# IXarea/LittleGAN

Measured on AMD Instinct MI355X. Metric: 128x128 CelebA-shaped images/sec (G+D+Adj step), higher is better.
Workload: dtype bf16; 1 GPU; C3: 128x128x3 synthetic CelebA, batch 256/GPU, bf16 MFMA conv/transposed-conv + Adjuster branch; global_batch=256, per_gpu_batch=256, image=128, cond_dim=40, parallelism=dp1, launch=eager launches

## Files before the change

include/littlegan_hip.h:

```cpp
#ifndef LITTLEGAN_HIP_H
#define LITTLEGAN_HIP_H
#include <stddef.h>

#ifdef __cplusplus
extern "C" {
#endif

#define LG_ABI_VERSION 1
#define LG_OK 0
#define LG_ERR_ARG (-1)
#define LG_ERR_LAUNCH (-2)
#define LG_ERR_UNSUPPORTED (-3)
#define LG_DT_F32 0
#define LG_DT_BF16 1

int lg_abi_version(void);
const char* lg_last_error(void);
const char* lg_last_kernel(void);
int lg_clear_kernel(void);

size_t lg_conv_pack_bytes(int cb, int cs, int dtype);
int lg_conv_pack(const float* w, void* pack, int cb, int cs, int dtype, void* stream);

int lg_conv2d_s2_fwd(const float* x, const void* pack, const float* bias, float* y, int B, int Hs, int Ws, int cb,
// ... 110 lines not shown
int lg_instnorm_leaky_bwd_drop(const float* x, const float* stats, const void* g, int g_is_bf16, float* dx, void* dx16,
                               float* dgamma, float* dbeta, float* db, int C, void* workspace, size_t ws_bytes, int B,
                               long long L, float alpha, int accumulate, const long long* key, int call, int level, int r0,
                               float rate, void* stream);
int lg_instnorm_leaky_bwd_z16_drop(const void* z16, const float* stats, const void* g, int g_is_bf16, float* dx, void* dx16,
                                   float* dgamma, float* dbeta, float* db, int C, const void* partials, int nparts_in,
                                   void* workspace, size_t ws_bytes, int B, long long L, float alpha, int accumulate,
                                   const long long* key, int call, int level, int r0, float rate, void* stream);

int lg_convT_s1_tanh_bwd_nf(const float* x, const void* x16, const float* dpre, const void* pack, void* dx16, float* dw,
                            float* db, void* workspace, size_t ws_bytes, int B, int H, int W, int cb, int cs, int accumulate,
                            int dtype, const void* z16, const float* stats, float alpha, void* part, size_t part_bytes,
                            int* nparts, void* stream);

int lg_dense_fwd(const float* x, const float* w, const float* bias, float* y, int B, int K, int N, void* stream);
int lg_dense_wgrad(const float* x, const float* dy, float* dw, float* db, int B, int K, int N, int accumulate,
                   void* stream);
int lg_dense_dgrad(const float* dy, const float* w, float* dx, int B, int K, int N, void* stream);
int lg_concat_cols(const float* a, int ka, const float* c, int kc, float* out, int B, void* stream);
int lg_adj_conditions(const float* first, const float* second, float* t, float* u, int B, int c, void* stream);
size_t lg_heads_fwd_workspace_bytes(int B, int K, int c);
int lg_heads_fwd(const float* x, const float* wpr, const float* bpr, const float* wc, const float* bc, float* p,
                 void* workspace, size_t ws_bytes, int B, int K, int c, void* stream);
int lg_heads_dgrad(const float* dz, const float* wpr, const float* wc, float* dx, int B, int K, int c, void* stream);
int lg_heads_wgrad(const float* x, const float* dz, float* dwpr, float* dbpr, float* dwc, float* dbc, int B, int K,
                   int c, int accumulate, void* stream);

int lg_bce_heads_loss_fwd_bwd(const float* p, const float* t_c, float t_pr, float w_pr, float w_c, float* loss,
                              float* dz, int B, int c, int accumulate, void* stream);
size_t lg_l1_workspace_bytes(void);
int lg_l1_tanh_loss_fwd_bwd(const float* t, const float* img, const float* g_in, float* dpre, float* loss,
                            void* workspace, size_t ws_bytes, long long n, float lambda, int accumulate, void* stream);

int lg_clip_adam_update(float* w, const float* g, float* m, float* v, long long n, const float* state, float lr,
                        float b1, float b2, float eps, float clip, float gscale, void* stream);
int lg_adam_advance(float* state, float b1, float b2, void* stream);
int lg_axpby(float* y, const float* x, float a, float b, long long n, void* stream);

int lg_clip_adam_ema_update(float* w, const float* g, float* m, float* v, float* ema, long long n, long long lo, long long hi,
// ... 68 lines not shown
```

littlegan_amd/_lib.py:

```python
from __future__ import annotations

import ctypes as C
import os

_HERE = os.path.dirname(os.path.abspath(__file__))
LIB_PATH = os.path.join(_HERE, "liblittlegan_hip.so")

DT_F32, DT_BF16 = 0, 1

P, I, L, F, Z = C.c_void_p, C.c_int, C.c_longlong, C.c_float, C.c_size_t

SIGNATURES = {
    "lg_abi_version": (I, []),
    "lg_last_error": (C.c_char_p, []),
    "lg_conv_pack_bytes": (Z, [I, I, I]),
    "lg_conv_pack": (I, [P, P, I, I, I, P]),
    "lg_conv2d_s2_fwd": (I, [P, P, P, P, I, I, I, I, I, I, P]),
    "lg_conv_stats_workspace_bytes": (Z, [I, I, I, I, I]),
    "lg_conv_fwd_stats_fused": (I, [I, I, I, I, I, I, I]),
    "lg_conv2d_s2_fwd_stats": (I, [P, P, P, P, P, P, I, I, I, I, I, I, P, Z, P, P]),
    "lg_conv2d_s2_dgrad_m16": (I, [P, P, P, P, P, I, I, I, I, I, I, P]),
    "lg_conv2d_s2_wgrad_m16": (I, [P, P, P, P, P, P, Z, I, I, I, I, I, I, I, P]),
    "lg_conv2d_s2_dgrad": (I, [P, P, P, I, I, I, I, I, I, P]),
    "lg_conv2d_s2_wgrad": (I, [P, P, P, P, Z, I, I, I, I, I, I, I, P]),
# ... 35 lines not shown
    "lg_instnorm_leaky_bwd_z16_p": (I, [P, P, P, I, P, P, P, P, P, I, P, I, P, Z, I, L, I, I, F, I, P]),
    "lg_conv2d_s2_dgrad_nf": (I, [P, P, P, I, I, I, I, I, P, P, F, P, Z, P, P]),
    "lg_convT_s2_dgrad_nf": (I, [P, P, P, I, I, I, I, I, P, P, F, P, Z, P, P]),
    "lg_convT_s2_dgrad_bn_supported": (I, [I, I, I, I, I]),
    "lg_convT_s2_dgrad_bn": (I, [P, P, P, F, P, P, I, I, I, I, I, P, P, F, P, Z, P, P]),
    "lg_instnorm_bwd_coef": (I, [P, P, I, P, I, L, P]),
    "lg_dropout_key": (I, [P, L, L, P]),
    "lg_dropout_mask": (I, [P, I, I, I, I, L, F, P, P]),
    "lg_instnorm_leaky_apply_drop": (I, [P, P, P, P, I, L, F, P, I, I, I, F, P]),
    "lg_instnorm_leaky_apply_z16_drop": (I, [P, P, P, P, I, L, F, P, I, I, I, F, P]),
    "lg_instnorm_leaky_apply_z16_p_drop": (I, [P, P, I, P, P, P, P, P, I, L, F, P, I, I, I, F, P]),
    "lg_instnorm_leaky_bwd_drop": (I, [P, P, P, I, P, P, P, P, P, I, P, Z, I, L, F, I, P, I, I, I, F, P]),
    "lg_instnorm_leaky_bwd_z16_drop": (I, [P, P, P, I, P, P, P, P, P, I, P, I, P, Z, I, L, F, I, P, I, I, I, F, P]),
    "lg_convT_s1_tanh_bwd_nf": (I, [P, P, P, P, P, P, P, P, Z, I, I, I, I, I, I, I, P, P, F, P, Z, P, P]),
    "lg_dense_fwd": (I, [P, P, P, P, I, I, I, P]),
    "lg_dense_wgrad": (I, [P, P, P, P, I, I, I, I, P]),
    "lg_dense_dgrad": (I, [P, P, P, I, I, I, P]),
    "lg_concat_cols": (I, [P, I, P, I, P, I, P]),
    "lg_adj_conditions": (I, [P, P, P, P, I, I, P]),
    "lg_heads_fwd_workspace_bytes": (Z, [I, I, I]),
    "lg_heads_fwd": (I, [P, P, P, P, P, P, P, Z, I, I, I, P]),
    "lg_heads_dgrad": (I, [P, P, P, P, I, I, I, P]),
    "lg_heads_wgrad": (I, [P, P, P, P, P, P, I, I, I, I, P]),
    "lg_bce_heads_loss_fwd_bwd": (I, [P, P, F, F, F, P, P, I, I, I, P]),
    "lg_l1_workspace_bytes": (Z, []),
    "lg_l1_tanh_loss_fwd_bwd": (I, [P, P, P, P, P, P, Z, L, F, I, P]),
    "lg_clip_adam_update": (I, [P, P, P, P, L, P, F, F, F, F, F, F, P]),
    "lg_adam_advance": (I, [P, F, F, P]),
    "lg_axpby": (I, [P, P, F, F, L, P]),
    "lg_clip_adam_ema_update": (I, [P, P, P, P, P, L, L, L, P, P, F, F, F, F, F, F, F, P]),
    "lg_ema_advance": (I, [P, P]),
    "lg_swap_f32": (I, [P, P, L, P]),
    "lg_philox4x32": (I, [P, I, L, L, P]),
    "lg_randn": (I, [P, L, F, F, L, L, P]),
    "lg_augment_workspace_bytes": (Z, [I]),
    "lg_augment": (I, [P, P, I, I, I, P, F, F, F, F, L, L, P, Z, P]),
    "lg_fid_stats_workspace_bytes": (Z, [L, I]),
# ... 70 lines not shown
```

littlegan_amd/csrc/dense.hip:

```cpp
#include "lg_common.h"

namespace {

template <int TB>
__global__ __launch_bounds__(256) void dense_fwd_kernel(const float* __restrict__ x, const float* __restrict__ w,
                                                        const float* __restrict__ bias, float* __restrict__ y, int B,
                                                        int K, int N) {
  extern __shared__ float xs[];
  const int b0 = blockIdx.y * TB;
  for (int i = threadIdx.x; i < TB * K; i += 256) {
    const int b = i / K, k = i - b * K;
    xs[i] = (b0 + b < B) ? x[(long long)(b0 + b) * K + k] : 0.f;
  }
  __syncthreads();
  const int n = (blockIdx.x * 256 + threadIdx.x) * 4;
  if (n >= N) return;
  f32x4 acc[TB];
  const f32x4 bv = bias ? *reinterpret_cast<const f32x4*>(bias + n) : f32x4{0.f, 0.f, 0.f, 0.f};
#pragma unroll
  for (int b = 0; b < TB; ++b) acc[b] = bv;
  for (int k = 0; k < K; ++k) {
    const f32x4 wv = *reinterpret_cast<const f32x4*>(w + (long long)k * N + n);
#pragma unroll
    for (int b = 0; b < TB; ++b) acc[b] += xs[b * K + k] * wv;
// ... 128 lines not shown
  LG_CHECK_ARG(x && w && y, "lg_dense_fwd: null pointer");
  LG_CHECK_ARG(B > 0 && K > 0 && K <= 1024 && N > 0 && N % 4 == 0, "lg_dense_fwd: bad shape B=%d K=%d N=%d", B, K, N);
  {
    const int rc = lg_dense_fwd_mfma_try(x, w, bias, y, B, K, N, stream);
    if (rc != LG_ERR_UNSUPPORTED) return rc;
  }
  constexpr int TB = 8;
  dim3 grid(lg_cdiv(N, 1024), lg_cdiv(B, TB));
  hipLaunchKernelGGL(dense_fwd_kernel<TB>, grid, dim3(256), TB * K * sizeof(float), (hipStream_t)stream, x, w, bias, y,
                     B, K, N);
  LG_CHECK_LAUNCH("lg_dense_fwd");
  lg_note_kernel("dense_fwd_kernel");
  return LG_OK;
}

extern "C" int lg_dense_wgrad(const float* x, const float* dy, float* dw, float* db, int B, int K, int N,
                              int accumulate, void* stream) {
  LG_CHECK_ARG(x && dy && dw, "lg_dense_wgrad: null pointer");
  LG_CHECK_ARG(B > 0 && K > 0 && N > 0 && N % 4 == 0, "lg_dense_wgrad: bad shape B=%d K=%d N=%d", B, K, N);
  {
    const int rc = lg_dense_wgrad_mfma_try(x, dy, dw, db, B, K, N, accumulate, stream);
    if (rc != LG_ERR_UNSUPPORTED) return rc;
  }
  constexpr int KT = 16;
  const size_t lds = ((size_t)((B * KT + 3) / 4) * 4 + (size_t)(KT + 1) * 64 * 4) * sizeof(float);
  LG_CHECK_ARG(lds <= 160 * 1024, "lg_dense_wgrad: batch %d too large for the LDS staging of x", B);
  static bool attr_set = false;
  if (!attr_set) {
    (void)hipFuncSetAttribute(reinterpret_cast<const void*>(dense_wgrad_kernel<KT>), hipFuncAttributeMaxDynamicSharedMemorySize, 160 * 1024);
    attr_set = true;
// ... 17 lines not shown
```

littlegan_amd/csrc/heads.hip:

```cpp
#include "lg_common.h"

namespace {

constexpr int HC_MAX = 40;

__device__ __forceinline__ float head_w(const float* __restrict__ wpr, const float* __restrict__ wc, int k, int j, int c) {
  return j == 0 ? wpr[k] : wc[(long long)k * c + (j - 1)];
}

constexpr int FS = 16;
constexpr int FKC = 256;

__global__ __launch_bounds__(256) void heads_fwd_kernel(const float* __restrict__ x, const float* __restrict__ wpr,
                                                        const float* __restrict__ wc, float* __restrict__ part, int B,
                                                        int K, int c) {
  __shared__ __attribute__((aligned(16))) float xs[FS][FKC];
  __shared__ float sred[4][FS][64];
  const int lane = threadIdx.x & 63, wid = threadIdx.x >> 6;
  const int b0 = blockIdx.y * FS, k0 = blockIdx.x * FKC;
  const bool act = lane <= c;
#pragma unroll
  for (int i = 0; i < FS * FKC / 4 / 256; ++i) {
    const int q = threadIdx.x + 256 * i, b = q / (FKC / 4), k4 = (q % (FKC / 4)) * 4;
    f32x4 v = {0.f, 0.f, 0.f, 0.f};
// ... 25 lines not shown
  for (int i = threadIdx.x; i < FS * 64; i += 256) {
    const int s = i >> 6, j = i & 63;
    if (j <= c && b0 + s < B)
      part[((long long)blockIdx.x * B + b0 + s) * (c + 1) + j] = (sred[0][s][j] + sred[1][s][j]) + (sred[2][s][j] + sred[3][s][j]);
  }
}

__global__ __launch_bounds__(256) void heads_final_kernel(const float* __restrict__ part, const float* __restrict__ bpr,
                                                          const float* __restrict__ bc, float* __restrict__ p, int B,
                                                          int c, int nkc) {
  const int i = blockIdx.x * 256 + threadIdx.x;
  const int n = B * (c + 1);
  if (i >= n) return;
  const int j = i % (c + 1);
  float z = 0.f;
  for (int q = 0; q < nkc; ++q) z += part[(long long)q * n + i];
  z += j == 0 ? bpr[0] : bc[j - 1];
  p[i] = 1.f / (1.f + expf(-z));
}

constexpr int DB = 16;
__global__ __launch_bounds__(256) void heads_dgrad_kernel(const float* __restrict__ dz, const float* __restrict__ wpr,
                                                          const float* __restrict__ wc, float* __restrict__ dx, int B,
                                                          int K, int c) {
  extern __shared__ __attribute__((aligned(16))) float dsm[];
  const int cp = c | 1;
  float* sw = dsm;
  float* sdz = dsm + ((256 * cp + 3) / 4) * 4;
  const int b0 = blockIdx.y * DB, k0 = blockIdx.x * 256;
  const int kn = min(256, K - k0);
  {
// ... 129 lines not shown
                              void* stream) {
  LG_CHECK_ARG(dz && wpr && wc && dx, "lg_heads_dgrad: null pointer");
  LG_CHECK_ARG(B > 0 && K > 0 && c >= 1 && c <= HC_MAX, "lg_heads_dgrad: bad shape B=%d K=%d c=%d", B, K, c);
  {
    const int rc = lg_heads_dgrad_mfma_try(dz, wpr, wc, dx, B, K, c, stream);
    if (rc != LG_ERR_UNSUPPORTED) return rc;
  }
  dim3 grid(lg_cdiv(K, 256), lg_cdiv(B, DB));
  const size_t lds = (size_t)((256 * (c | 1) + 3) / 4 * 4 + DB * (c + 1)) * sizeof(float);
  hipLaunchKernelGGL(heads_dgrad_kernel, grid, dim3(256), lds, (hipStream_t)stream, dz, wpr, wc, dx, B, K, c);
  LG_CHECK_LAUNCH("lg_heads_dgrad");
  lg_note_kernel("heads_dgrad_kernel");
  return LG_OK;
}

extern "C" int lg_heads_wgrad(const float* x, const float* dz, float* dwpr, float* dbpr, float* dwc, float* dbc, int B,
                              int K, int c, int accumulate, void* stream) {
  LG_CHECK_ARG(x && dz && dwpr && dbpr && dwc && dbc, "lg_heads_wgrad: null pointer");
  LG_CHECK_ARG(B > 0 && K > 0 && K % 4 == 0 && c >= 1 && c <= HC_MAX, "lg_heads_wgrad: bad shape B=%d K=%d c=%d", B, K, c);
  {
    const int rc = lg_heads_wgrad_mfma_try(x, dz, dwpr, dbpr, dwc, dbc, B, K, c, accumulate, stream);
    if (rc != LG_ERR_UNSUPPORTED) return rc;
  }
  hipLaunchKernelGGL(heads_wgrad_kernel, dim3(lg_cdiv(K, WK)), dim3(256), 0, (hipStream_t)stream, x, dz, dwpr, dbpr,
                     dwc, dbc, B, K, c, accumulate);
  LG_CHECK_LAUNCH("lg_heads_wgrad");
  lg_note_kernel("heads_wgrad_kernel");
  return LG_OK;
}
```

littlegan_amd/csrc/skinny_mfma.hip:

```cpp
#include <stdlib.h>
#include "lg_common.h"

namespace {

__device__ __forceinline__ f32x16 mfma2(float a, float b, f32x16 c) { return __builtin_amdgcn_mfma_f32_32x32x2f32(a, b, c, 0, 0, 0); }
__device__ __forceinline__ f32x16 zero16() {
  f32x16 z;
#pragma unroll
  for (int e = 0; e < 16; ++e) z[e] = 0.f;
  return z;
}
struct HeadCol { const float* ptr; int stride; bool ok; };
__device__ __forceinline__ HeadCol head_col(const float* wpr, const float* wc, int j, int c) {
  HeadCol h;
  h.ok = j <= c;
  h.ptr = j == 0 ? wpr : wc + (h.ok ? j - 1 : 0);
  h.stride = j == 0 ? 1 : c;
  return h;
}

__global__ __launch_bounds__(256) void heads_fwd_mfma_kernel(const float* __restrict__ x, const float* __restrict__ wpr,
                                                             const float* __restrict__ wc, float* __restrict__ part, int B,
                                                             int K, int c) {
  __shared__ float sred[4][2][16][64];
  const int lane = threadIdx.x & 63, wid = threadIdx.x >> 6, r = lane & 31, h = lane >> 5;
  const int b0 = blockIdx.y * 32, kw = blockIdx.x * 512 + wid * 128 + 8 * h;
  const float* xr = x + (long long)(b0 + r) * K + kw;
  const HeadCol c0 = head_col(wpr, wc, r, c), c1 = head_col(wpr, wc, 32 + r, c);
  const bool two = c >= 32;
  f32x16 acc0 = zero16(), acc1 = zero16();
  constexpr int GU = 2;
  for (int g2 = 0; g2 < 8; g2 += GU) {
    f32x4 alo[GU], ahi[GU];
    float w0[GU][8], w1[GU][8];
// ... 112 lines not shown
    bw[s] = j <= c ? (j == 0 ? wpr[kt + r] : wc[(long long)(kt + r) * c + j - 1]) : 0.f;
  }
  __syncthreads();
  for (int t = 0; t < nmt; ++t) {
    const int mt = blockIdx.y + t * gridDim.y;
    const float* zr = sdz + (t * 32 + r) * cp + h;
    f32x16 acc = zero16();
#pragma unroll
    for (int s = 0; s < SMAX; ++s) acc = mfma2(2 * s + h <= c ? zr[2 * s] : 0.f, bw[s], acc);
    float* o = dx + (long long)(mt * 32 + 4 * h) * K + kt + r;
#pragma unroll
    for (int e = 0; e < 16; ++e) o[(long long)((e & 3) + 8 * (e >> 2)) * K] = acc[e];
  }
}

constexpr int SD = 72;
__global__ __launch_bounds__(256) void dense_fwd_mfma_kernel(const float* __restrict__ x, const float* __restrict__ w,
                                                             const float* __restrict__ bias, float* __restrict__ y, int B,
                                                             int K, int N) {
  extern __shared__ float sx[];
  const int lane = threadIdx.x & 63, wid = threadIdx.x >> 6, r = lane & 31, h = lane >> 5;
  const int n = blockIdx.x * 128 + wid * 32 + r, b0 = blockIdx.y * 32;
  const int nsteps = (K + 1) / 2, kp = K | 1;
  {
    const float* src = x + (long long)b0 * K;
    int row = threadIdx.x / K, col = threadIdx.x - row * K;
    const int dq = 256 / K, dr = 256 - dq * K;
    for (int i = threadIdx.x; i < 32 * K; i += 256) {
      sx[row * kp + col] = src[i];
      row += dq; col += dr;
// ... 10 lines not shown
#pragma unroll 4
  for (int s = 0; s < nsteps; s += 2) {
    const bool ok = 2 * s + h < K, ok2 = 2 * s + 2 + h < K;
    const float a = ok ? xr[2 * s] : 0.f, a2 = ok2 ? xr[2 * s + 2] : 0.f;
    const float b = ok ? wp[(long long)(2 * s) * N] : 0.f, b2 = ok2 ? wp[(long long)(2 * s + 2) * N] : 0.f;
    acc = mfma2(a, b, acc);
    acc2 = mfma2(a2, b2, acc2);
  }
#pragma unroll
  for (int e = 0; e < 16; ++e) acc[e] += acc2[e];
  float* o = y + (long long)(b0 + 4 * h) * N + n;
#pragma unroll
  for (int e = 0; e < 16; ++e) o[(long long)((e & 3) + 8 * (e >> 2)) * N] = acc[e];
}

template <int MT>
__global__ __launch_bounds__(256) void dense_wgrad_mfma_kernel(const float* __restrict__ x, const float* __restrict__ dy,
                                                               float* __restrict__ dw, float* __restrict__ db, int B, int K,
                                                               int N, int accumulate) {
  __shared__ float red[MT][16][64];
  __shared__ float rb[64];
  const int lane = threadIdx.x & 63, wid = threadIdx.x >> 6, r = lane & 31, h = lane >> 5;
  const int n = blockIdx.x * 32 + r;
  const int bq = B / 4, bs = wid * bq;
  f32x16 acc[MT];
#pragma unroll
  for (int m = 0; m < MT; ++m) acc[m] = zero16();
  float bsum = 0.f;
  const float* dp = dy + (long long)(bs + h) * N + n;
  const float* xp = x + (long long)(bs + h) * K + r;
// ... 31 lines not shown
      float* o = dw + (long long)k * N + blockIdx.x * 32 + rr;
      *o = (accumulate ? *o : 0.f) + red[m][e][hh * 32 + rr];
    }
  }
  if (db && threadIdx.x < 32) {
    float* o = db + blockIdx.x * 32 + threadIdx.x;
    *o = (accumulate ? *o : 0.f) + (rb[threadIdx.x] + rb[32 + threadIdx.x]);
  }
}

bool skinny_on() {
  static int on = -1;
  if (on < 0) on = lg_env_flag("LG_NO_SKINNY_MFMA") ? 0 : 1;
  return on == 1;
}

}

extern "C" int lg_heads_fwd_mfma_try(const float* x, const float* wpr, const float* wc, float* part, int B, int K, int c,
                                     int* nkc_out, void* stream) {
  if (!skinny_on() || B % 32 || K % 512 || c < 1 || c > 40) return LG_ERR_UNSUPPORTED;
  hipLaunchKernelGGL(heads_fwd_mfma_kernel, dim3(K / 512, B / 32), dim3(256), 0, (hipStream_t)stream, x, wpr, wc, part, B, K, c);
  LG_CHECK_LAUNCH("lg_heads_fwd(mfma)");
  lg_note_kernel("heads_fwd_mfma_kernel");
  *nkc_out = K / 512;
  return LG_OK;
}

extern "C" int lg_heads_wgrad_mfma_try(const float* x, const float* dz, float* dwpr, float* dbpr, float* dwc, float* dbc, int B,
                                       int K, int c, int accumulate, void* stream) {
  if (!skinny_on() || B % 64 || K % 32 || c < 1 || c > 40) return LG_ERR_UNSUPPORTED;
  hipLaunchKernelGGL(heads_wgrad_mfma_kernel, dim3(K / 32), dim3(256), 0, (hipStream_t)stream, x, dz, dwpr, dbpr, dwc, dbc, B, K, c,
                     accumulate);
  LG_CHECK_LAUNCH("lg_heads_wgrad(mfma)");
  lg_note_kernel("heads_wgrad_mfma_kernel");
  return LG_OK;
}

extern "C" int lg_heads_dgrad_mfma_try(const float* dz, const float* wpr, const float* wc, float* dx, int B, int K, int c,
                                       void* stream) {
  if (!skinny_on() || B % 32 || K % 128 || c < 1 || c > 40) return LG_ERR_UNSUPPORTED;
  const int mt = B / 32, gy = mt >= 8 ? 4 : (mt >= 2 ? 2 : 1);
  const size_t lds = (size_t)((mt + gy - 1) / gy) * 32 * ((c + 1) | 1) * sizeof(float);
  if (lds > 48 * 1024) return LG_ERR_UNSUPPORTED;
  hipLaunchKernelGGL(heads_dgrad_mfma_kernel, dim3(K / 128, gy), dim3(256), lds, (hipStream_t)stream, dz, wpr, wc, dx, B, K, c);
  LG_CHECK_LAUNCH("lg_heads_dgrad(mfma)");
  lg_note_kernel("heads_dgrad_mfma_kernel");
  return LG_OK;
}

extern "C" int lg_dense_fwd_mfma_try(const float* x, const float* w, const float* bias, float* y, int B, int K, int N,
                                     void* stream) {
  if (!skinny_on() || B % 32 || N % 128 || K < 1 || K > 2 * SD) return LG_ERR_UNSUPPORTED;
  hipLaunchKernelGGL(dense_fwd_mfma_kernel, dim3(N / 128, B / 32), dim3(256), (size_t)32 * (K | 1) * sizeof(float),
                     (hipStream_t)stream, x, w, bias, y, B, K, N);
  LG_CHECK_LAUNCH("lg_dense_fwd(mfma)");
  lg_note_kernel("dense_fwd_mfma_kernel");
  return LG_OK;
}

extern "C" int lg_dense_wgrad_mfma_try(const float* x, const float* dy, float* dw, float* db, int B, int K, int N, int accumulate,
                                       void* stream) {
// ... 13 lines not shown
```

littlegan_amd/model.py:

```python
from __future__ import annotations

import math
import zlib
from typing import Dict, List, Optional

import torch

from . import ops
from ._lib import DT_BF16, DT_F32


def _dtype_of(args) -> int:
    name = getattr(args, "mfma_dtype", "f32")
    if name not in ("f32", "bf16"):
        raise ValueError(f"mfma_dtype must be 'f32' or 'bf16', got {name!r}")
    return DT_BF16 if name == "bf16" else DT_F32


def _device_of(args):
    return torch.device(getattr(args, "device", "cuda"))


def _glorot(shape, gen, device):
    if len(shape) == 2:
# ... 114 lines not shown
                st = ops.stats_tensor(st)
                m = h if i == 4 else h16
            else:
                h16 = None
                h = m = ops.instnorm_apply(z, st, None, 0, 1, a, drop=drops[i - 1] if drops else None)
            outs.append(m if tails is None else (m, tails[i - 1]))
            saved.append((x, z, st, x16))
            x, x16, raw = h, h16, None
        if ctx is not None:
            ctx["enc"] = saved
            ctx["enc_maps"] = outs
            ctx["enc_drop"] = drops
        return outs

    def backward(self, ctx, g_last, need_wgrad: bool, need_input_grad: bool, rows: Optional[slice] = None,
                 wgrad_levels=None):
        a = self.args.leaky_alpha
        packs = self.packs()
        drops = ctx.get("enc_drop")
        r0 = 0
        if drops is not None and rows is not None:
            r0, _, step = rows.indices(ctx["enc"][0][1].shape[0])
            if step != 1:
                raise ValueError("Encoder.backward: contiguous row ranges only")
        masked = drops is not None and drops[0].active
        g_h = g_last
        levels = set(range(1, 5)) if (need_wgrad and wgrad_levels is None) else (set(wgrad_levels or ()) if need_wgrad else set())
        lowest = 1 if need_input_grad else (min(levels) if levels else 5)
        any_wgrad = need_wgrad
        nfp = None
        for i in range(4, lowest - 1, -1):
            need_wgrad = any_wgrad and i in levels
            cb, cs = self.chans[i - 1]
            x, z, st, x16 = ctx["enc"][i - 1]
            if need_wgrad and x is None and x16 is None:
                raise ValueError("Encoder.backward: this context was recorded with top_only=True (no normalised inputs kept): "
                                 "it cannot give weight gradients")
            if rows is not None:
                z, st = z[rows], st[rows]
                x = x[rows] if x is not None else None
                x16 = x16[rows] if x16 is not None else None
            dgm = self._g[f"norm{i}.gamma"] if need_wgrad else None
            dbt = self._g[f"norm{i}.beta"] if need_wgrad else None
            want_dx = i > lowest or (i == 1 and need_input_grad)
            m16 = self.dtype == DT_BF16
# ... 212 lines not shown


class _DenseNorm(_Module):

    def __init__(self, args, in_dim):
        super().__init__(args)
        self.in_dim = in_dim
        self.out_dim = args.init_dim ** 2 * args.conv_filter[0]
        self._add("dense.kernel", (in_dim, self.out_dim), "kernel")
        self._add("dense.bias", (self.out_dim,), "zeros")
        self._add("norm.gamma", (1,), "ones")
        self._add("norm.beta", (1,), "zeros")

    def __call__(self, x, ctx: Optional[dict] = None, skip=None, want16: bool = False):
        a = self.args.leaky_alpha
        u = ops.dense_fwd(x, self._w["dense.kernel"], self._w["dense.bias"])
        st = ops.instnorm_stats(u, self._w["norm.gamma"], self._w["norm.beta"], 1, a)
        w16 = torch.empty(u.shape, dtype=torch.bfloat16, device=u.device) if want16 else None
        if isinstance(skip, tuple):
            b1 = skip[0].shape[0]
            w = torch.empty_like(u)
            for lo, hi, sk in ((0, b1, skip[0]), (b1, u.shape[0], skip[1])):
                ops.instnorm_apply(u[lo:hi], st[lo:hi], sk.reshape(hi - lo, -1), 1, 0, a, out=w[lo:hi],
                                   out16=w16[lo:hi] if want16 else None)
        else:
            w = ops.instnorm_apply(u, st, skip.reshape(u.shape) if skip is not None else None, 1, 0, a, out16=w16)
        if ctx is not None:
            ctx["dn"] = (x, u, st)
        shp = (-1, self.args.init_dim, self.args.init_dim, self.args.conv_filter[0])
        return w.view(shp), (w16.view(shp) if want16 else None)

    def backward(self, ctx, g):
# ... 107 lines not shown

    def __call__(self, inputs, ctx: Optional[dict] = None):
        p = self.forward_packed(inputs, ctx)
        return p[:, :1], p[:, 1:]

    def backward(self, ctx, dz, need_wgrad: bool, need_input_grad: bool, rows: Optional[slice] = None, train_range=None):
        lo, hi = train_range if train_range is not None else (0, 20)
        heads = need_wgrad and lo <= 16 and hi >= 20
        levels = [i for i in range(1, 5) if lo <= 4 * (i - 1) and 4 * i <= hi] if need_wgrad else []
        x = ctx["heads_x"] if rows is None else ctx["heads_x"][rows]
        if heads:
            ops.heads_wgrad(x, dz, self._g["dense_pr.kernel"], self._g["dense_pr.bias"], self._g["dense_cond.kernel"],
                            self._g["dense_cond.bias"])
        if not levels and not need_input_grad:
            return None
        dx = ops.heads_dgrad(dz, self._w["dense_pr.kernel"], self._w["dense_cond.kernel"])
        i, f = self.args.init_dim, self.args.conv_filter[0]
        return self.encoder.backward(ctx, dx.view(-1, i, i, f), bool(levels), need_input_grad, rows, wgrad_levels=levels)

    def gradient_penalty(self, image, gp_weight: float, loss=None, gp_loss=None, train_range=None):
        lo, hi = train_range if train_range is not None else (0, 20)
        heads = lo <= 16 and hi >= 20
        levels = [i for i in range(1, 5) if lo <= 4 * (i - 1) and 4 * i <= hi]
        ctx: dict = {}
        p = self.forward_packed(image, ctx)
        B = image.shape[0]
        i, f = self.args.init_dim, self.args.conv_filter[0]
        wpr = self._w["dense_pr.kernel"]
        g_top = ops.gp_heads_seed(p, wpr)
        g0, rec = self.encoder.backward_recorded(ctx, g_top.view(B, i, i, f))
        u0, r = ops.gp_seed(g0, gp_weight, loss, gp_loss)
        u4, uz2 = self.encoder.gp_sweep(ctx, rec, u0, levels, min(levels) if levels else 5)
        _, g2 = ops.gp_heads_2nd(p, wpr, ctx["heads_x"], u4.view(B, -1), dwpr=self._g["dense_pr.kernel"] if heads else None,
# ... 104 lines not shown
```

littlegan_amd/ops.py:

```python
from __future__ import annotations

import torch

from . import _lib
from ._lib import DT_BF16, DT_F32, check

_WS = {}
_WS_RETIRED = []
_WS_PINNED = False
NSTAT = 8


class Profile:
    enabled = False
    records = []
    after_conv = None

    @classmethod
    def start(cls):
        cls.records = []
        cls.enabled = True

    @classmethod
    def stop(cls):
# ... 621 lines not shown
    return out


def dense_fwd(x, w, bias, out=None):
    B, K = x.shape
    N = w.shape[1]
    _chk(x, name="x")
    _chk(w, (K, N), "w")
    if out is None:
        out = torch.empty(B, N, dtype=torch.float32, device=x.device)
    _chk(out, (B, N), "out")
    check(_lib.load().lg_dense_fwd(_p(x), _p(w), _p(bias), _p(out), B, K, N, _stream()), "lg_dense_fwd")
    return out


def dense_wgrad(x, dy, dw, db, accumulate=False):
    B, K = x.shape
    N = dy.shape[1]
    _chk(x, name="x")
    _chk(dy, (B, N), "dy")
    _chk(dw, (K, N), "dw")
    check(_lib.load().lg_dense_wgrad(_p(x), _p(dy), _p(dw), _p(db), B, K, N, int(accumulate), _stream()),
          "lg_dense_wgrad")


def concat_cols(a, c, out=None):
    B, ka = a.shape
    kc = c.shape[1]
    _chk(a, name="a")
    _chk(c, (B, kc), "c")
# ... 39 lines not shown
    ws = workspace(int(lib.lg_heads_fwd_workspace_bytes(B, K, c)), x.device, "small")
    check(lib.lg_heads_fwd(_p(x), _p(wpr), _p(bpr), _p(wc), _p(bc), _p(out), _p(ws), ws.numel(), B, K, c, _stream()),
          "lg_heads_fwd")
    return out


def heads_dgrad(dz, wpr, wc, out=None):
    B = dz.shape[0]
    K, c = wc.shape
    _chk(dz, (B, 1 + c), "dz")
    if out is None:
        out = torch.empty(B, K, dtype=torch.float32, device=dz.device)
    _chk(out, (B, K), "out")
    check(_lib.load().lg_heads_dgrad(_p(dz), _p(wpr), _p(wc), _p(out), B, K, c, _stream()), "lg_heads_dgrad")
    return out


def heads_wgrad(x, dz, dwpr, dbpr, dwc, dbc, accumulate=False):
    B, K = x.shape
    c = dwc.shape[1]
    _chk(x, name="x")
    _chk(dz, (B, 1 + c), "dz")
    _chk(dwpr, (K, 1), "dwpr")
    _chk(dwc, (K, c), "dwc")
    check(_lib.load().lg_heads_wgrad(_p(x), _p(dz), _p(dwpr), _p(dbpr), _p(dwc), _p(dbc), B, K, c, int(accumulate),
                                     _stream()), "lg_heads_wgrad")


def bce_heads_loss(p, t_c, t_pr, w_pr, w_c, loss, dz, accumulate):
    B, J = p.shape
# ... 477 lines not shown
```

Measured before the change: 24290 images/sec.

## Fuse instnorm moments into dense fwd and norm-bwd partials into heads dgrad

Adds a dense forward MFMA kernel that computes per-row leaky/instnorm moment partials (count, mean, M2 in double) in its epilogue, so the generator's first norm no longer needs a separate stats pass. Adds a heads dgrad variant that also reads the bf16 encoder level-4 pre-activation and stats, producing norm-backward partial sums that are passed to the encoder backward. The heads fwd reduction loop is batched into 16-wide loads. The aim is fewer kernel launches and fewer re-reads of activations, at the cost of extra register pressure, double-precision shuffles and new workspaces.

```diff
diff --git a/include/littlegan_hip.h b/include/littlegan_hip.h
--- a/include/littlegan_hip.h
+++ b/include/littlegan_hip.h
@@ -148,6 +148,10 @@
                             int* nparts, void* stream);
 
 int lg_dense_fwd(const float* x, const float* w, const float* bias, float* y, int B, int K, int N, void* stream);
+int lg_dense_fwd_mom_supported(int B, int K, int N);
+size_t lg_dense_fwd_mom_workspace_bytes(int B, int N);
+int lg_dense_fwd_mom(const float* x, const float* w, const float* bias, float* y, int B, int K, int N, float alpha, void* mom,
+                     size_t mom_bytes, int* nparts, void* stream);
 int lg_dense_wgrad(const float* x, const float* dy, float* dw, float* db, int B, int K, int N, int accumulate,
                    void* stream);
 int lg_dense_dgrad(const float* dy, const float* w, float* dx, int B, int K, int N, void* stream);
@@ -157,6 +161,11 @@
 int lg_heads_fwd(const float* x, const float* wpr, const float* bpr, const float* wc, const float* bc, float* p,
                  void* workspace, size_t ws_bytes, int B, int K, int c, void* stream);
 int lg_heads_dgrad(const float* dz, const float* wpr, const float* wc, float* dx, int B, int K, int c, void* stream);
+int lg_set_top_fuse(int on);
+int lg_heads_dgrad_nf_supported(int B, int K, int c, int C);
+size_t lg_heads_dgrad_nf_workspace_bytes(int B, int K);
+int lg_heads_dgrad_nf(const float* dz, const float* wpr, const float* wc, float* dx, int B, int K, int c, int C, const void* z16,
+                      const float* stats, float alpha, void* part, size_t part_bytes, int* nparts, void* stream);
 int lg_heads_wgrad(const float* x, const float* dz, float* dwpr, float* dbpr, float* dwc, float* dbc, int B, int K,
                    int c, int accumulate, void* stream);
 
diff --git a/littlegan_amd/_lib.py b/littlegan_amd/_lib.py
--- a/littlegan_amd/_lib.py
+++ b/littlegan_amd/_lib.py
@@ -73,6 +73,9 @@
     "lg_instnorm_leaky_bwd_z16_drop": (I, [P, P, P, I, P, P, P, P, P, I, P, I, P, Z, I, L, F, I, P, I, I, I, F, P]),
     "lg_convT_s1_tanh_bwd_nf": (I, [P, P, P, P, P, P, P, P, Z, I, I, I, I, I, I, I, P, P, F, P, Z, P, P]),
     "lg_dense_fwd": (I, [P, P, P, P, I, I, I, P]),
+    "lg_dense_fwd_mom_supported": (I, [I, I, I]),
+    "lg_dense_fwd_mom_workspace_bytes": (Z, [I, I]),
+    "lg_dense_fwd_mom": (I, [P, P, P, P, I, I, I, F, P, Z, P, P]),
     "lg_dense_wgrad": (I, [P, P, P, P, I, I, I, I, P]),
     "lg_dense_dgrad": (I, [P, P, P, I, I, I, P]),
     "lg_concat_cols": (I, [P, I, P, I, P, I, P]),
@@ -80,6 +83,10 @@
     "lg_heads_fwd_workspace_bytes": (Z, [I, I, I]),
     "lg_heads_fwd": (I, [P, P, P, P, P, P, P, Z, I, I, I, P]),
     "lg_heads_dgrad": (I, [P, P, P, P, I, I, I, P]),
+    "lg_set_top_fuse": (I, [I]),
+    "lg_heads_dgrad_nf_supported": (I, [I, I, I, I]),
+    "lg_heads_dgrad_nf_workspace_bytes": (Z, [I, I]),
+    "lg_heads_dgrad_nf": (I, [P, P, P, P, I, I, I, I, P, P, F, P, Z, P, P]),
     "lg_heads_wgrad": (I, [P, P, P, P, P, P, I, I, I, I, P]),
     "lg_bce_heads_loss_fwd_bwd": (I, [P, P, F, F, F, P, P, I, I, I, P]),
     "lg_l1_workspace_bytes": (Z, []),
diff --git a/littlegan_amd/csrc/dense.hip b/littlegan_amd/csrc/dense.hip
--- a/littlegan_amd/csrc/dense.hip
+++ b/littlegan_amd/csrc/dense.hip
@@ -166,6 +166,26 @@
   return LG_OK;
 }
 
+extern "C" int lg_dense_fwd_mom_mfma_try(const float* x, const float* w, const float* bias, float* y, int B, int K, int N,
+                                         double* mom, float alpha, void* stream);
+
+extern "C" size_t lg_dense_fwd_mom_workspace_bytes(int B, int N) {
+  if (B <= 0 || N <= 0) return 0;
+  return (size_t)B * (size_t)lg_cdiv(N, 128) * 3 * sizeof(double);
+}
+
+extern "C" int lg_dense_fwd_mom(const float* x, const float* w, const float* bias, float* y, int B, int K, int N, float alpha,
+                                void* mom, size_t mom_bytes, int* nparts, void* stream) {
+  LG_CHECK_ARG(x && w && y && mom && nparts, "lg_dense_fwd_mom: null pointer");
+  LG_CHECK_ARG(B > 0 && K > 0 && K <= 1024 && N > 0 && N % 4 == 0, "lg_dense_fwd_mom: bad shape B=%d K=%d N=%d", B, K, N);
+  LG_CHECK_ARG(mom_bytes >= lg_dense_fwd_mom_workspace_bytes(B, N), "lg_dense_fwd_mom: workspace too small (%zu bytes)", mom_bytes);
+  *nparts = 0;
+  const int rc = lg_dense_fwd_mom_mfma_try(x, w, bias, y, B, K, N, (double*)mom, alpha, stream);
+  if (rc == LG_OK) *nparts = N / 128;
+  if (rc != LG_ERR_UNSUPPORTED) return rc;
+  return lg_dense_fwd(x, w, bias, y, B, K, N, stream);
+}
+
 extern "C" int lg_dense_wgrad(const float* x, const float* dy, float* dw, float* db, int B, int K, int N,
                               int accumulate, void* stream) {
   LG_CHECK_ARG(x && dy && dw, "lg_dense_wgrad: null pointer");
diff --git a/littlegan_amd/csrc/heads.hip b/littlegan_amd/csrc/heads.hip
--- a/littlegan_amd/csrc/heads.hip
+++ b/littlegan_amd/csrc/heads.hip
@@ -63,7 +63,14 @@
   if (i >= n) return;
   const int j = i % (c + 1);
   float z = 0.f;
-  for (int q = 0; q < nkc; ++q) z += part[(long long)q * n + i];
+  for (int q0 = 0; q0 < nkc; q0 += 16) {
+    float v[16];
+#pragma unroll
+    for (int u = 0; u < 16; ++u) v[u] = q0 + u < nkc ? part[(long long)(q0 + u) * n + i] : 0.f;
+#pragma unroll
+    for (int u = 0; u < 16; ++u)
+      if (q0 + u < nkc) z += v[u];
+  }
   z += j == 0 ? bpr[0] : bc[j - 1];
   p[i] = 1.f / (1.f + expf(-z));
 }
@@ -223,6 +230,27 @@
   return LG_OK;
 }
 
+extern "C" int lg_heads_dgrad_nf_mfma_try(const float* dz, const float* wpr, const float* wc, float* dx, int B, int K, int c, int C,
+                                          const void* z16, const float* stats, float alpha, double* part, void* stream);
+
+extern "C" size_t lg_heads_dgrad_nf_workspace_bytes(int B, int K) {
+  if (B <= 0 || K <= 0) return 0;
+  return (size_t)B * (size_t)lg_cdiv(K, 128) * 2 * sizeof(double);
+}
+
+extern "C" int lg_heads_dgrad_nf(const float* dz, const float* wpr, const float* wc, float* dx, int B, int K, int c, int C,
+                                 const void* z16, const float* stats, float alpha, void* part, size_t part_bytes, int* nparts,
+                                 void* stream) {
+  LG_CHECK_ARG(dz && wpr && wc && dx && z16 && stats && part && nparts, "lg_heads_dgrad_nf: null pointer");
+  LG_CHECK_ARG(B > 0 && K > 0 && c >= 1 && c <= HC_MAX && C > 0, "lg_heads_dgrad_nf: bad shape B=%d K=%d c=%d C=%d", B, K, c, C);
+  LG_CHECK_ARG(part_bytes >= lg_heads_dgrad_nf_workspace_bytes(B, K), "lg_heads_dgrad_nf: workspace too small (%zu bytes)", part_bytes);
+  *nparts = 0;
+  const int rc = lg_heads_dgrad_nf_mfma_try(dz, wpr, wc, dx, B, K, c, C, z16, stats, alpha, (double*)part, stream);
+  if (rc == LG_OK) *nparts = K / 128;
+  if (rc != LG_ERR_UNSUPPORTED) return rc;
+  return lg_heads_dgrad(dz, wpr, wc, dx, B, K, c, stream);
+}
+
 extern "C" int lg_heads_wgrad(const float* x, const float* dz, float* dwpr, float* dbpr, float* dwc, float* dbc, int B,
                               int K, int c, int accumulate, void* stream) {
   LG_CHECK_ARG(x && dz && dwpr && dbpr && dwc && dbc, "lg_heads_wgrad: null pointer");
diff --git a/littlegan_amd/csrc/skinny_mfma.hip b/littlegan_amd/csrc/skinny_mfma.hip
--- a/littlegan_amd/csrc/skinny_mfma.hip
+++ b/littlegan_amd/csrc/skinny_mfma.hip
@@ -18,6 +18,22 @@
   h.stride = j == 0 ? 1 : c;
   return h;
 }
+
+
+template <int N>
+__device__ __forceinline__ void rs_step(double (&v)[16], int r, int o) {
+  const bool up = (r & o) != 0;
+#pragma unroll
+  for (int i = 0; i < N; ++i) {
+    const double keep = up ? v[i + N] : v[i], send = up ? v[i] : v[i + N];
+    v[i] = keep + __shfl_xor(send, o, 64);
+  }
+}
+__device__ __forceinline__ double rs16(double (&v)[16], int r) {
+  rs_step<8>(v, r, 16); rs_step<4>(v, r, 8); rs_step<2>(v, r, 4); rs_step<1>(v, r, 2);
+  return v[0] + __shfl_xor(v[0], 1, 64);
+}
+__device__ __forceinline__ int acc_row(int e, int h) { return (e & 3) + 8 * (e >> 2) + 4 * h; }
 
 __global__ __launch_bounds__(256) void heads_fwd_mfma_kernel(const float* __restrict__ x, const float* __restrict__ wpr,
                                                              const float* __restrict__ wc, float* __restrict__ part, int B,
@@ -160,6 +176,78 @@
   }
 }
 
+
+__global__ __launch_bounds__(256) void heads_dgrad_nf_mfma_kernel(const float* __restrict__ dz, const float* __restrict__ wpr,
+                                                                  const float* __restrict__ wc, float* __restrict__ dx, int B,
+                                                                  int K, int c, const unsigned short* __restrict__ z,
+                                                                  const float* __restrict__ stats, double* __restrict__ part,
+                                                                  float alpha) {
+  constexpr int SMAX = 21;
+  extern __shared__ float sdz[];
+  __shared__ f32x4 sst[2][32];
+  __shared__ double sred[2][4][32][2];
+  const int lane = threadIdx.x & 63, wid = threadIdx.x >> 6, r = lane & 31, h = lane >> 5;
+  const int kt = blockIdx.x * 128 + wid * 32;
+  const int cp = (c + 1) | 1, nmt = (B / 32 - blockIdx.y + gridDim.y - 1) / gridDim.y, nparts = K / 128;
+  for (int t = 0; t < nmt; ++t) {
+    const float* src = dz + (long long)(blockIdx.y + t * gridDim.y) * 32 * (c + 1);
+    for (int i = threadIdx.x; i < 32 * (c + 1); i += 256) {
+      const int row = i / (c + 1), j = i - row * (c + 1);
+      sdz[(t * 32 + row) * cp + j] = src[i];
+    }
+  }
+  float bw[SMAX];
+#pragma unroll
+  for (int s = 0; s < SMAX; ++s) {
+    const int j = 2 * s + h;
+    bw[s] = j <= c ? (j == 0 ? wpr[kt + r] : wc[(long long)(kt + r) * c + j - 1]) : 0.f;
+  }
+  if (threadIdx.x < 32) {
+    const float* sp = stats + (long long)(blockIdx.y * 32 + threadIdx.x) * 8;
+    sst[0][threadIdx.x] = f32x4{sp[0], sp[4], sp[2], sp[3]};
+  }
+  __syncthreads();
+  for (int t = 0; t < nmt; ++t) {
+    const int mt = blockIdx.y + t * gridDim.y, pb = t & 1;
+    if (t + 1 < nmt && threadIdx.x < 32) {
+      const float* sp = stats + (long long)((mt + gridDim.y) * 32 + threadIdx.x) * 8;
+      sst[pb ^ 1][threadIdx.x] = f32x4{sp[0], sp[4], sp[2], sp[3]};
+    }
+    const unsigned short* zp = z + (long long)(mt * 32 + 4 * h) * K + kt + r;
+    unsigned short zv[16];
+#pragma unroll
+    for (int e = 0; e < 16; ++e) zv[e] = zp[(long long)((e & 3) + 8 * (e >> 2)) * K];
+    const float* zr = sdz + (t * 32 + r) * cp + h;
+    f32x16 acc = zero16();
+#pragma unroll
+    for (int s = 0; s < SMAX; ++s) acc = mfma2(2 * s + h <= c ? zr[2 * s] : 0.f, bw[s], acc);
+    float* o = dx + (long long)(mt * 32 + 4 * h) * K + kt + r;
+#pragma unroll
+    for (int e = 0; e < 16; ++e) o[(long long)((e & 3) + 8 * (e >> 2)) * K] = acc[e];
+    double v1[16], v2[16];
+#pragma unroll
+    for (int e = 0; e < 16; ++e) {
+      const f32x4 sr = sst[pb][acc_row(e, h)];
+      const float zf = __builtin_bit_cast(float, (unsigned)zv[e] << 16);
+      const float cc = (zf - sr[0]) - sr[1];
+      const float p = (sr[2] * cc + sr[3] > 0.f) ? acc[e] : alpha * acc[e];
+      v1[e] = (double)p;
+      v2[e] = (double)(p * cc);
+    }
+    const double s1 = rs16(v1, r), s2 = rs16(v2, r);
+    if (!(r & 1)) {
+      const int row = acc_row(r >> 1, h);
+      sred[pb][wid][row][0] = s1; sred[pb][wid][row][1] = s2;
+    }
+    __syncthreads();
+    if (threadIdx.x < 64) {
+      const int row = threadIdx.x >> 1, q = threadIdx.x & 1;
+      part[((long long)(mt * 32 + row) * nparts + blockIdx.x) * 2 + q] =
+          (sred[pb][0][row][q] + sred[pb][1][row][q]) + (sred[pb][2][row][q] + sred[pb][3][row][q]);
+    }
+  }
+}
+
 constexpr int SD = 72;
 __global__ __launch_bounds__(256) void dense_fwd_mfma_kernel(const float* __restrict__ x, const float* __restrict__ w,
                                                              const float* __restrict__ bias, float* __restrict__ y, int B,
@@ -200,6 +288,65 @@
   for (int e = 0; e < 16; ++e) o[(long long)((e & 3) + 8 * (e >> 2)) * N] = acc[e];
 }
 
+__global__ __launch_bounds__(256) void dense_fwd_mom_mfma_kernel(const float* __restrict__ x, const float* __restrict__ w,
+                                                                 const float* __restrict__ bias, float* __restrict__ y, int B,
+                                                                 int K, int N, double* __restrict__ mom, float alpha) {
+  extern __shared__ float sx[];
+  __shared__ double swv[4][32];
+  __shared__ double smean[32];
+  const int lane = threadIdx.x & 63, wid = threadIdx.x >> 6, r = lane & 31, h = lane >> 5;
+  const int n = blockIdx.x * 128 + wid * 32 + r, b0 = blockIdx.y * 32;
+  const int nsteps = (K + 1) / 2, kp = K | 1;
+  {
+    const float* src = x + (long long)b0 * K;
+    int row = threadIdx.x / K, col = threadIdx.x - row * K;
+    const int dq = 256 / K, dr = 256 - dq * K;
+    for (int i = threadIdx.x; i < 32 * K; i += 256) {
+      sx[row * kp + col] = src[i];
+      row += dq; col += dr;
+      if (col >= K) { col -= K; ++row; }
+    }
+  }
+  __syncthreads();
+  const float* xr = sx + r * kp + h;
+  const float* wp = w + (long long)h * N + n;
+  const float bv = bias ? bias[n] : 0.f;
+  f32x16 acc, acc2 = zero16();
+#pragma unroll
+  for (int e = 0; e < 16; ++e) acc[e] = bv;
+#pragma unroll 4
+  for (int s = 0; s < nsteps; s += 2) {
+    const bool ok = 2 * s + h < K, ok2 = 2 * s + 2 + h < K;
+    const float a = ok ? xr[2 * s] : 0.f, a2 = ok2 ? xr[2 * s + 2] : 0.f;
+    const float b = ok ? wp[(long long)(2 * s) * N] : 0.f, b2 = ok2 ? wp[(long long)(2 * s + 2) * N] : 0.f;
+    acc = mfma2(a, b, acc);
+    acc2 = mfma2(a2, b2, acc2);
+  }
+#pragma unroll
+  for (int e = 0; e < 16; ++e) acc[e] += acc2[e];
+  float* o = y + (long long)(b0 + 4 * h) * N + n;
+#pragma unroll
+  for (int e = 0; e < 16; ++e) o[(long long)((e & 3) + 8 * (e >> 2)) * N] = acc[e];
+  double v[16];
+#pragma unroll
+  for (int e = 0; e < 16; ++e) { acc[e] = lg_leaky(acc[e], alpha); v[e] = (double)acc[e]; }
+  const double sw = rs16(v, r);
+  if (!(r & 1)) swv[wid][acc_row(r >> 1, h)] = sw;
+  __syncthreads();
+  if (threadIdx.x < 32) smean[threadIdx.x] = ((swv[0][threadIdx.x] + swv[1][threadIdx.x]) + (swv[2][threadIdx.x] + swv[3][threadIdx.x])) / 128.0;
+  __syncthreads();
+#pragma unroll
+  for (int e = 0; e < 16; ++e) { const double d = (double)acc[e] - smean[acc_row(e, h)]; v[e] = d * d; }
+  const double qw = rs16(v, r);
+  if (!(r & 1)) swv[wid][acc_row(r >> 1, h)] = qw;
+  __syncthreads();
+  if (threadIdx.x < 32) {
+    double* rec = mom + ((long long)(b0 + threadIdx.x) * (N / 128) + blockIdx.x) * 3;
+    rec[0] = 128.0; rec[1] = smean[threadIdx.x];
+    rec[2] = (swv[0][threadIdx.x] + swv[1][threadIdx.x]) + (swv[2][threadIdx.x] + swv[3][threadIdx.x]);
+  }
+}
+
 template <int MT>
 __global__ __launch_bounds__(256) void dense_wgrad_mfma_kernel(const float* __restrict__ x, const float* __restrict__ dy,
                                                                float* __restrict__ dw, float* __restrict__ db, int B, int K,
@@ -261,6 +408,16 @@
   if (on < 0) on = lg_env_flag("LG_NO_SKINNY_MFMA") ? 0 : 1;
   return on == 1;
 }
+int g_top_fuse = 1;
+bool top_fuse_on() { return g_top_fuse != 0; }
+bool heads_dgrad_geo(int B, int K, int c, int* gy_out, size_t* lds_out) {
+  if (!skinny_on() || B % 32 || K % 128 || c < 1 || c > 40) return false;
+  const int mt = B / 32, gy = mt >= 8 ? 4 : (mt >= 2 ? 2 : 1);
+  const size_t lds = (size_t)((mt + gy - 1) / gy) * 32 * ((c + 1) | 1) * sizeof(float);
+  if (lds > 48 * 1024) return false;
+  *gy_out = gy; *lds_out = lds;
+  return true;
+}
 
 }
 
@@ -286,13 +443,49 @@
 
 extern "C" int lg_heads_dgrad_mfma_try(const float* dz, const float* wpr, const float* wc, float* dx, int B, int K, int c,
                                        void* stream) {
-  if (!skinny_on() || B % 32 || K % 128 || c < 1 || c > 40) return LG_ERR_UNSUPPORTED;
-  const int mt = B / 32, gy = mt >= 8 ? 4 : (mt >= 2 ? 2 : 1);
-  const size_t lds = (size_t)((mt + gy - 1) / gy) * 32 * ((c + 1) | 1) * sizeof(float);
-  if (lds > 48 * 1024) return LG_ERR_UNSUPPORTED;
+  int gy;
+  size_t lds;
+  if (!heads_dgrad_geo(B, K, c, &gy, &lds)) return LG_ERR_UNSUPPORTED;
   hipLaunchKernelGGL(heads_dgrad_mfma_kernel, dim3(K / 128, gy), dim3(256), lds, (hipStream_t)stream, dz, wpr, wc, dx, B, K, c);
   LG_CHECK_LAUNCH("lg_heads_dgrad(mfma)");
   lg_note_kernel("heads_dgrad_mfma_kernel");
+  return LG_OK;
+}
+
+extern "C" int lg_set_top_fuse(int on) {
+  const int old = g_top_fuse;
+  g_top_fuse = on ? 1 : 0;
+  return old;
+}
+
+extern "C" int lg_heads_dgrad_nf_supported(int B, int K, int c, int C) {
+  int gy;
+  size_t lds;
+  return (top_fuse_on() && C > 0 && C % 32 == 0 && K % C == 0 && heads_dgrad_geo(B, K, c, &gy, &lds)) ? 1 : 0;
+}
+extern "C" int lg_dense_fwd_mom_supported(int B, int K, int N) {
+  return (top_fuse_on() && skinny_on() && B > 0 && B % 32 == 0 && N > 0 && N % 128 == 0 && K >= 1 && K <= 2 * SD) ? 1 : 0;
+}
+
+extern "C" int lg_heads_dgrad_nf_mfma_try(const float* dz, const float* wpr, const float* wc, float* dx, int B, int K, int c, int C,
+                                          const void* z16, const float* stats, float alpha, double* part, void* stream) {
+  int gy;
+  size_t lds;
+  if (!lg_heads_dgrad_nf_supported(B, K, c, C) || !heads_dgrad_geo(B, K, c, &gy, &lds)) return LG_ERR_UNSUPPORTED;
+  hipLaunchKernelGGL(heads_dgrad_nf_mfma_kernel, dim3(K / 128, gy), dim3(256), lds, (hipStream_t)stream, dz, wpr, wc, dx, B, K, c,
+                     (const unsigned short*)z16, stats, part, alpha);
+  LG_CHECK_LAUNCH("lg_heads_dgrad_nf(mfma)");
+  lg_note_kernel("heads_dgrad_nf_mfma_kernel");
+  return LG_OK;
+}
+
+extern "C" int lg_dense_fwd_mom_mfma_try(const float* x, const float* w, const float* bias, float* y, int B, int K, int N,
+                                         double* mom, float alpha, void* stream) {
+  if (!lg_dense_fwd_mom_supported(B, K, N)) return LG_ERR_UNSUPPORTED;
+  hipLaunchKernelGGL(dense_fwd_mom_mfma_kernel, dim3(N / 128, B / 32), dim3(256), (size_t)32 * (K | 1) * sizeof(float),
+                     (hipStream_t)stream, x, w, bias, y, B, K, N, mom, alpha);
+  LG_CHECK_LAUNCH("lg_dense_fwd_mom(mfma)");
+  lg_note_kernel("dense_fwd_mom_mfma_kernel");
   return LG_OK;
 }
 
diff --git a/littlegan_amd/model.py b/littlegan_amd/model.py
--- a/littlegan_amd/model.py
+++ b/littlegan_amd/model.py
@@ -152,7 +152,7 @@
         return outs
 
     def backward(self, ctx, g_last, need_wgrad: bool, need_input_grad: bool, rows: Optional[slice] = None,
-                 wgrad_levels=None):
+                 wgrad_levels=None, partials=None):
         a = self.args.leaky_alpha
         packs = self.packs()
         drops = ctx.get("enc_drop")
@@ -166,7 +166,7 @@
         levels = set(range(1, 5)) if (need_wgrad and wgrad_levels is None) else (set(wgrad_levels or ()) if need_wgrad else set())
         lowest = 1 if need_input_grad else (min(levels) if levels else 5)
         any_wgrad = need_wgrad
-        nfp = None
+        nfp = None if masked else partials
         for i in range(4, lowest - 1, -1):
             need_wgrad = any_wgrad and i in levels
             cb, cs = self.chans[i - 1]
@@ -409,8 +409,8 @@
 
     def __call__(self, x, ctx: Optional[dict] = None, skip=None, want16: bool = False):
         a = self.args.leaky_alpha
-        u = ops.dense_fwd(x, self._w["dense.kernel"], self._w["dense.bias"])
-        st = ops.instnorm_stats(u, self._w["norm.gamma"], self._w["norm.beta"], 1, a)
+        u, mom = ops.dense_fwd_moments(x, self._w["dense.kernel"], self._w["dense.bias"], self._w["norm.gamma"], self._w["norm.beta"], a)
+        st = ops.stats_tensor(mom) if mom is not None else ops.instnorm_stats(u, self._w["norm.gamma"], self._w["norm.beta"], 1, a)
         w16 = torch.empty(u.shape, dtype=torch.bfloat16, device=u.device) if want16 else None
         if isinstance(skip, tuple):
             b1 = skip[0].shape[0]
@@ -548,9 +548,18 @@
                             self._g["dense_cond.bias"])
         if not levels and not need_input_grad:
             return None
-        dx = ops.heads_dgrad(dz, self._w["dense_pr.kernel"], self._w["dense_cond.kernel"])
+        z4, st4 = ctx["enc"][3][1], ctx["enc"][3][2]
+        nfp = None
+        if z4.dtype == torch.bfloat16:
+            if rows is not None:
+                z4, st4 = z4[rows], st4[rows]
+            dx, nfp = ops.heads_dgrad_nf(dz, self._w["dense_pr.kernel"], self._w["dense_cond.kernel"],
+                                         (z4, ops.stats_tensor(st4), self.args.leaky_alpha))
+        else:
+            dx = ops.heads_dgrad(dz, self._w["dense_pr.kernel"], self._w["dense_cond.kernel"])
         i, f = self.args.init_dim, self.args.conv_filter[0]
-        return self.encoder.backward(ctx, dx.view(-1, i, i, f), bool(levels), need_input_grad, rows, wgrad_levels=levels)
+        return self.encoder.backward(ctx, dx.view(-1, i, i, f), bool(levels), need_input_grad, rows, wgrad_levels=levels,
+                                     partials=nfp)
 
     def gradient_penalty(self, image, gp_weight: float, loss=None, gp_loss=None, train_range=None):
         lo, hi = train_range if train_range is not None else (0, 20)
diff --git a/littlegan_amd/ops.py b/littlegan_amd/ops.py
--- a/littlegan_amd/ops.py
+++ b/littlegan_amd/ops.py
@@ -659,6 +659,25 @@
     return out
 
 
+def dense_fwd_moments(x, w, bias, gamma, beta, alpha, out=None):
+    import ctypes
+    B, K = x.shape
+    N = w.shape[1]
+    _chk(x, name="x")
+    _chk(w, (K, N), "w")
+    if out is None:
+        out = torch.empty(B, N, dtype=torch.float32, device=x.device)
+    _chk(out, (B, N), "out")
+    lib = _lib.load()
+    if not lib.lg_dense_fwd_mom_supported(B, K, N):
+        return dense_fwd(x, w, bias, out), None
+    ws = workspace(int(lib.lg_dense_fwd_mom_workspace_bytes(B, N)), x.device, "statpart")
+    nparts = ctypes.c_int(0)
+    check(lib.lg_dense_fwd_mom(_p(x), _p(w), _p(bias), _p(out), B, K, N, float(alpha), _p(ws), ws.numel(), ctypes.addressof(nparts),
+                               _stream()), "lg_dense_fwd_mom")
+    return out, (Moments(ws, nparts.value, gamma, beta, B) if nparts.value > 0 else None)
+
+
 def dense_wgrad(x, dy, dw, db, accumulate=False):
     B, K = x.shape
     N = dy.shape[1]
@@ -728,6 +747,28 @@
     _chk(out, (B, K), "out")
     check(_lib.load().lg_heads_dgrad(_p(dz), _p(wpr), _p(wc), _p(out), B, K, c, _stream()), "lg_heads_dgrad")
     return out
+
+
+def heads_dgrad_nf(dz, wpr, wc, fuse, out=None):
+    import ctypes
+    B = dz.shape[0]
+    K, c = wc.shape
+    _chk(dz, (B, 1 + c), "dz")
+    z16, st, alpha = fuse
+    if z16.dtype != torch.bfloat16 or not z16.is_contiguous() or z16.dim() != 4 or z16.shape[0] != B or z16.numel() != B * K:
+        raise ValueError("heads_dgrad_nf: fuse z16 must be the contiguous bf16 [B, H, W, C] conv output under the heads")
+    _chk(st, (B, NSTAT), "fuse stats")
+    if out is None:
+        out = torch.empty(B, K, dtype=torch.float32, device=dz.device)
+    _chk(out, (B, K), "out")
+    lib = _lib.load()
+    if not lib.lg_heads_dgrad_nf_supported(B, K, c, int(z16.shape[-1])):
+        return heads_dgrad(dz, wpr, wc, out), None
+    ws = workspace(int(lib.lg_heads_dgrad_nf_workspace_bytes(B, K)), dz.device, "nfpart")
+    npo = ctypes.c_int(0)
+    check(lib.lg_heads_dgrad_nf(_p(dz), _p(wpr), _p(wc), _p(out), B, K, c, int(z16.shape[-1]), _p(z16), _p(st), float(alpha), _p(ws),
+                                ws.numel(), ctypes.addressof(npo), _stream()), "lg_heads_dgrad_nf")
+    return out, (NormPartials(ws, npo.value, alpha, z16.shape) if npo.value > 0 else None)
 
 
 def heads_wgrad(x, dz, dwpr, dbpr, dwc, dbc, accumulate=False):
```

Measured after the change: 24310 images/sec, median of 5. About the same (+0.1%).
